# Amanda-Zheng/MR-GNAS

Measured on AMD Instinct MI355X. Metric: million edges/sec per supernet fwd+bwd step (FB15k-237, dim=200), higher is better.
Workload: dtype f32

## Files before the change

### include/mrgnas.h

```cpp
#ifndef MRGNAS_H
#define MRGNAS_H

#include <stdint.h>

#ifdef __cplusplus
extern "C" {
#endif

#define MRG_ABI_VERSION 23

#define MRG_OK            0
#define MRG_E_NULLPTR    -1
#define MRG_E_SHAPE      -2
#define MRG_E_ENUM       -3
#define MRG_E_WORKSPACE  -4

#define MRG_COMPOSE_MULT 0
#define MRG_COMPOSE_SUB  1
#define MRG_COMPOSE_ADD  2
#define MRG_REDUCE_SUM   0
#define MRG_REDUCE_MEAN  1
#define MRG_REDUCE_MAX   2
#define MRG_GCS_SUB      0
#define MRG_GCS_MUL      1
// ... 31 lines not shown
int mrg_gate_fwd(const float *s, const float *s_in, const float *norm, const float *uvc,
                 float *out, int64_t b0, int64_t b1, int64_t M, int D, float scale, void *stream);
int64_t mrg_gate_bwd_workspace_bytes(int64_t M, int D);
int mrg_gate_bwd(const float *gout, const float *s, const float *s_in, const float *norm,
                 const float *uvc, float *gs, float *gs_in, float *d_uvc, void *ws,
                 int64_t b0, int64_t b1, int64_t M, int D, float scale, void *stream);
int mrg_gate_row_fwd(const float *s, const float *s_in, const float *norm, const float *uvc, float *fvec, float *hvec,
                     int64_t b0, int64_t b1, int64_t M, int D, float scale, void *stream);
int64_t mrg_gate_row_colsum_blocks(int64_t b0, int64_t b1, int64_t M, int D, int vec4);
int mrg_gate_row_fwd_colsum(const float *s, const float *s_in, const float *norm, const float *uvc, float *fvec, float *hvec,
                            int64_t b0, int64_t b1, int64_t M, int D, float scale, void *stream, double *colsum, int64_t colsum_blocks);
int mrg_gate_row_bwd(const float *q, const float *hvec, const float *s, const float *s_in, const float *uvc, float *gs_in, float *d_uvc,
                     void *ws, int64_t b0, int64_t b1, int64_t M, int D, void *stream);
int mrg_gate_row_bwd_acc(const float *q, const float *hvec, const float *s, const float *s_in, const float *uvc, float *gs_in, float *d_uvc,
                         void *ws, int64_t b0, int64_t b1, int64_t M, int D, void *stream, const float *total);

int64_t mrg_seg_reduce_workspace_bytes(int64_t n_slots, int D);
int mrg_seg_reduce_fwd(int mode, const float *msg, const float *self_rows,
                       const int32_t *eid,
                       const int32_t *chunk_node, const int32_t *chunk_start, const int32_t *chunk_end,
                       const int32_t *chunk_slot, int64_t n_chunks,
                       const int32_t *hub_node, const int32_t *hub_first, const int32_t *hub_count, int64_t n_hubs,
                       int64_t n_slots, const int32_t *in_degree,
                       float *out, int32_t *arg, void *ws,
                       int64_t N, int D, void *stream);
int mrg_seg_reduce_bwd(int mode, const float *gout, const int32_t *dst, const int32_t *in_degree,
                       const int32_t *arg, float *gmsg, float *gself, const float *relu_src,
                       int64_t E, int64_t N, int D, void *stream);
int mrg_seg_reduce_bwd_ordered(int mode, const float *gout, const int32_t *dst, const int32_t *in_degree, const int32_t *arg,
                               float *gmsg, float *gself, const float *relu_src, const unsigned *relu_bits, const int32_t *order,
// ... 144 lines not shown
                                 int64_t b0, int64_t b1, int64_t M, int D, void *stream, double *colsum, int64_t colsum_blocks);
int mrg_dense_filter_dz3(int kind, const float *g, const float *s, const float *gate, const float *norm, float scale_edge,
                         float scale_self, float *dz, float *gs, int64_t b1, int64_t M, int D, void *stream);
int64_t mrg_linear_bwd_input3_workspace_bytes(int K, int Nout);
int mrg_linear_bwd_input3(const float *gY, const float *const *W, float *gX, void *ws, int64_t b0, int64_t b1, int64_t M,
                          int K, int Nout, int ldw, int accumulate, void *stream);
int64_t mrg_linear_bwd_input3_pair_workspace_bytes(int K, int Nout);
int mrg_linear_bwd_input3_pair(const float *gY1, const float *gY2, const float *const *W1, const float *const *W2, float *gX,
                               void *ws, int64_t b0, int64_t b1, int64_t M, int K, int Nout, int ldw, int accumulate,
                               void *stream);
int mrg_linear_bwd_input3_acc2(const float *gY, const float *const *W, float *gX, void *ws, int64_t b0, int64_t b1, int64_t M,
                               int K, int Nout, int ldw, int accumulate, void *stream, const float *total);
int mrg_linear_bwd_input3_pair_acc2(const float *gY1, const float *gY2, const float *const *W1, const float *const *W2, float *gX,
                                    void *ws, int64_t b0, int64_t b1, int64_t M, int K, int Nout, int ldw, int accumulate,
                                    void *stream, const float *total);
int64_t mrg_linear_bwd_weight3_workspace_bytes(int64_t b0, int64_t b1, int64_t M, int K1, int K2, int Nout);
int mrg_linear_bwd_weight3(const float *gY, const float *X1, const float *X2, float *const *gW, float *const *gbias, void *ws,
                           int64_t b0, int64_t b1, int64_t M, int K1, int K2, int Nout, void *stream);
int mrg_dense_filter_dz(int kind, const float *g, const float *s, const float *gate, const float *rowscale,
                        float scale, float *dz, float *gs, int64_t rows, int D, void *stream);

int64_t mrg_build_graph_workspace_bytes(int64_t T);
int mrg_build_graph(const int64_t *triples, int64_t T, int64_t N, int R, int sorted,
                    const float *deg_norm_table, int64_t table_len,
                    int64_t *src, int64_t *dst, int64_t *etype, float *norm, int32_t *in_degree,
                    int32_t *src32, int32_t *dst32, int32_t *etype32, int32_t *max_degree,
                    void *ws, int64_t ws_bytes, void *stream);

int64_t mrg_plan_workspace_bytes(int64_t E, int64_t nseg, int span);
int mrg_span_plan_build(const int32_t *seg, int64_t E, int64_t nseg, int span, int snap,
// ... 176 lines not shown
```

### mr-gnas_amd/_lib.py

```python
import ctypes
import os
import re

import torch

_HERE = os.path.dirname(os.path.abspath(__file__))
LIB_PATH = os.environ.get("MRG_LIB_PATH") or os.path.join(_HERE, "lib", "libmrgnas_hip.so")
HEADER_PATH = os.path.join(os.path.dirname(_HERE), "include", "mrgnas.h")

ABI_VERSION = 23


class MrgnasLibraryError(RuntimeError):
    pass


class MrgnasError(RuntimeError):
    """A C-ABI call returned a non-zero code."""


_P, _I, _L, _F = ctypes.c_void_p, ctypes.c_int, ctypes.c_int64, ctypes.c_float

SIGNATURES = {
    "mrg_abi_version": (_I, []),
# ... 10 lines not shown
    "mrg_gate_bwd_workspace_bytes": (_L, [_L, _I]),
    "mrg_gate_bwd": (_I, [_P, _P, _P, _P, _P, _P, _P, _P, _P, _L, _L, _L, _I, _F, _P]),
    "mrg_seg_reduce_workspace_bytes": (_L, [_L, _I]),
    "mrg_seg_reduce_fwd": (_I, [_I, _P, _P, _P, _P, _P, _P, _P, _L, _P, _P, _P, _L, _L, _P, _P, _P, _P, _L, _I, _P]),
    "mrg_seg_reduce_bwd": (_I, [_I, _P, _P, _P, _P, _P, _P, _P, _L, _L, _I, _P]),
    "mrg_fused_gcs": (_I, [_I, _P, _P, _P, _P, _P, _P, _P, _P, _P, _P, _L, _P, _P, _P, _L, _L, _P, _P, _P, _L, _I, _P]),
    "mrg_span_gcs": (_I, [_I, _P, _P, _P, _P, _L, _I, _P, _P, _L, _P, _P, _P, _L, _L, _P, _P, _P, _L, _I, _P]),
    "mrg_sum_buffers": (_I, [_P, _I, _P, _L, _I, _P]),
    "mrg_sum_rows_gather": (_I, [_P, _I, _P, _P, _P, _L, _L, _I, _P, _P]),
    "mrg_distmult_score": (_I, [_P, _P, _P, _P, _P, _P, _L, _I, _P]),
    "mrg_gate_row_fwd": (_I, [_P, _P, _P, _P, _P, _P, _L, _L, _L, _I, _F, _P]),
    "mrg_gate_row_colsum_blocks": (_L, [_L, _L, _L, _I, _I]),
    "mrg_gate_row_fwd_colsum": (_I, [_P, _P, _P, _P, _P, _P, _L, _L, _L, _I, _F, _P, _P, _L]),
    "mrg_gate_row_bwd": (_I, [_P, _P, _P, _P, _P, _P, _P, _P, _L, _L, _L, _I, _P]),
    "mrg_gate_row_bwd_acc": (_I, [_P, _P, _P, _P, _P, _P, _P, _P, _L, _L, _L, _I, _P, _P]),
    "mrg_mix_workspace_bytes": (_L, [_I, _I]),
    "mrg_mix_colstats": (_I, [_P, _I, _L, _I, _P, _P, _P, _P]),
    "mrg_mix_finalize_fwd": (_I, [_P, _P, _P, _P, _P, _I, ctypes.c_double, _I, _F, _F, _P, _P]),
    "mrg_mix_stats_coef": (_I, [_P, _P, _P, _P, _P, _I, _L, ctypes.c_double, _I, _F, _F, _P, _P, _P, _P]),
    "mrg_zero_workspace_bytes": (_L, [_I]),
    "mrg_zero_colstats": (_I, [_P, _P, _P, _P, _P, _I, _L, _I, _P, _P, _P]),
    "mrg_zero_stats_coef": (_I, [_P, _P, _P, _P, _P, _I, _P, _P, _P, _P, _L, ctypes.c_double, _I, _F, _F, _P, _P, _P, _P]),
    "mrg_zero_fwd": (_I, [_P, _P, _P, _P, _P, _I, _P, _P, _P, _L, _I, _P, _P]),
    "mrg_zero_bwd_reduce": (_I, [_P, _P, _P, _P, _P, _P, _I, _P, _P, _P, _P, _L, _I, _P, _P]),
    "mrg_zero_bwd_apply": (_I, [_P, _P, _P, _P, _P, _P, _I, _P, _P, _P, _P, _P, _L, _I, _P, _P]),
    "mrg_mix_fwd": (_I, [_P, _I, _P, _P, _P, _P, _L, _I, _P, _P]),
    "mrg_mix_bwd_reduce": (_I, [_P, _P, _I, _P, _P, _P, _P, _L, _I, _P, _P]),
    "mrg_mix_finalize_bwd": (_I, [_P, _I, ctypes.c_double, _I, _P, _P, _P, _P, _P, _P]),
    "mrg_mix_bwd_apply": (_I, [_P, _P, _P, _I, _P, _P, _P, _P, _P, _P, _P, _P, _P, _P, _P, _P, _P, _L, _I, _P, _P]),
    "mrg_dense_filter_fwd": (_I, [_I, _P, _P, _P, _P, _P, _F, _P, _P, _P, _L, _I, _P]),
# ... 14 lines not shown
    "mrg_adam_step": (_I, [_P, _P, _P, _P, _L, _P, _P, _P, _L, _P, _P, _P, ctypes.c_double, ctypes.c_double, _F, _F, _P]),
    "mrg_act_grad_transpose": (_I, [_P, _P, _P, _L, _L, _I, _P]),
    "mrg_wgrad_set_variant": (_I, [_I]),
    "mrg_linear_fwd": (_I, [_P, _P, _P, _P, _P, _L, _I, _I, _I, _P]),
    "mrg_dense_filter3_workspace_bytes": (_L, [_I, _I]),
    "mrg_dense_filter_fwd3": (_I, [_I, _P, _P, _P, _P, _P, _F, _F, _P, _P, _P, _L, _L, _L, _I, _P]),
    "mrg_dense_filter3_colsum_blocks": (_L, [_I, _L, _L, _L, _I, _I]),
    "mrg_dense_filter_fwd3_colsum": (_I, [_I, _P, _P, _P, _P, _P, _F, _F, _P, _P, _P, _L, _L, _L, _I, _P, _P, _L]),
    "mrg_dense_filter_dz3": (_I, [_I, _P, _P, _P, _P, _F, _F, _P, _P, _L, _L, _I, _P]),
    "mrg_linear_bwd_input3_workspace_bytes": (_L, [_I, _I]),
    "mrg_linear_bwd_input3": (_I, [_P, _P, _P, _P, _L, _L, _L, _I, _I, _I, _I, _P]),
    "mrg_linear_bwd_input3_acc2": (_I, [_P, _P, _P, _P, _L, _L, _L, _I, _I, _I, _I, _P, _P]),
    "mrg_linear_bwd_input3_pair_workspace_bytes": (_L, [_I, _I]),
    "mrg_linear_bwd_input3_pair": (_I, [_P, _P, _P, _P, _P, _P, _L, _L, _L, _I, _I, _I, _I, _P]),
    "mrg_linear_bwd_input3_pair_acc2": (_I, [_P, _P, _P, _P, _P, _P, _L, _L, _L, _I, _I, _I, _I, _P, _P]),
    "mrg_linear_bwd_weight3_workspace_bytes": (_L, [_L, _L, _L, _I, _I, _I]),
    "mrg_linear_bwd_weight3": (_I, [_P, _P, _P, _P, _P, _P, _L, _L, _L, _I, _I, _I, _P]),
    "mrg_linear_relu_segsum_fwd": (_I, [_P, _P, _P, _P, _P, _P, _P, _P, _L, _I, _I, _P]),
    "mrg_seg_reduce_heads_fwd": (_I, [_I, _P, _P, _P, _P, _P, _P, _P, _L, _P, _P, _P, _L, _L, _P, _P, _P, _L, _I, _P]),
    "mrg_seg_reduce_bwd_bits": (_I, [_I, _P, _P, _P, _P, _P, _P, _L, _L, _I, _P]),
    "mrg_seg_reduce_bwd_ordered": (_I, [_I, _P, _P, _P, _P, _P, _P, _P, _P, _P, _L, _L, _I, _P]),
    "mrg_linear_relu_segmax_workspace_bytes": (_L, [_L, _I, _I]),
    "mrg_linear_relu_segmax_fwd": (_I, [_P, _P, _P, _P, _P, _P, _P, _P, _P, _P, _L, _L, _I, _I, _P]),
    "mrg_linear_bwd_input_workspace_bytes": (_L, [_I, _I]),
    "mrg_linear_bwd_input": (_I, [_P, _P, _P, _P, _L, _I, _I, _I, _I, _P]),
    "mrg_linear_bwd_input_acc2": (_I, [_P, _P, _P, _P, _L, _I, _I, _I, _I, _P, _P]),
    "mrg_linear_bwd_weight_workspace_bytes": (_L, [_L, _I, _I]),
    "mrg_linear_bwd_weight": (_I, [_P, _P, _P, _P, _P, _P, _L, _I, _I, _I, _P]),
    "mrg_linear_bwd_weight_share": (_I, [_P, _P, _P, _P, _P, _P, _L, _I, _I, _I, _I, _P]),
    "mrg_build_graph_workspace_bytes": (_L, [_L]),
# ... 255 lines not shown
```

### mr-gnas_amd/csrc/gate.hip

```cpp
#include "common.hpp"

namespace mrg {

struct SegPlan {
  int64_t lo[3], hi[3];
  int blk[4];
};

static SegPlan make_plan(int64_t b0, int64_t b1, int64_t M, int grid) {
  SegPlan p;
  p.lo[0] = 0;  p.hi[0] = b0;
  p.lo[1] = b0; p.hi[1] = b1;
  p.lo[2] = b1; p.hi[2] = M;
  int nseg = 0;
  for (int s = 0; s < 3; ++s) nseg += (p.hi[s] > p.lo[s]);
  int spare = grid - nseg;
  p.blk[0] = 0;
  for (int s = 0; s < 3; ++s) {
    int64_t rows = p.hi[s] - p.lo[s];
    int nb = rows > 0 ? 1 + (int)((double)spare * (double)rows / (double)M) : 0;
    p.blk[s + 1] = p.blk[s] + nb;
  }
  return p;
}
// ... 362 lines not shown
  float* mine = red + rw * (2 * WIDTH + 1);
#pragma unroll
  for (int k = 0; k < KMAX; ++k) {
    int c = sl + k * LPR;
#pragma unroll
    for (int j = 0; j < VEC; ++j) {
      mine[c * VEC + j] = du[k][j];
      mine[WIDTH + c * VEC + j] = dvv[k][j];
    }
  }
  if (sl == 0) mine[2 * WIDTH] = (float)dc;
  __syncthreads();
  float* dst = ws + (int64_t)b * ld;
  for (int t = threadIdx.x; t < ld; t += MRG_BLOCK) {
    int srcidx = t < D ? t : ((HAS_IN && t < 2 * D) ? WIDTH + (t - D) : (t == cidx ? 2 * WIDTH : -1));
    double acc = 0.0;
    if (srcidx >= 0) {
#pragma unroll
      for (int q = 0; q < RPB; ++q) acc += (double)red[q * (2 * WIDTH + 1) + srcidx];
    }
    dst[t] = (float)acc;
  }
}

__global__ void gate_reduce_k(const float* __restrict__ ws, float* __restrict__ d_uvc, SegPlan p, int ld) {
  int seg = blockIdx.y;
  int t = blockIdx.x * blockDim.x + threadIdx.x;
  if (t >= ld) return;
  double acc = 0.0;
  for (int b = p.blk[seg]; b < p.blk[seg + 1]; ++b) acc += (double)ws[(int64_t)b * ld + t];
// ... 230 lines not shown
extern "C" int64_t mrg_gate_row_colsum_blocks(int64_t b0, int64_t b1, int64_t M, int D, int vec4) {
  if (D <= 0 || M <= 0 || b0 < 0 || b1 < b0 || M < b1) return 0;
  RowGeom g = row_geom(D, vec4 != 0);
  if (!g.ok || g.kmax != 1 || (vec4 && g.vec != 4)) return 0;
  SegPlan p;
  return gate_row_plan(b0, b1, M, g.lpr, &p);
}

extern "C" int mrg_gate_row_fwd_colsum(const float* s, const float* s_in, const float* norm, const float* uvc, float* fvec, float* hvec,
                                       int64_t b0, int64_t b1, int64_t M, int D, float scale, void* stream, double* colsum, int64_t colsum_blocks) {
  if (!colsum) return MRG_E_NULLPTR;
  return gate_row_fwd(s, s_in, norm, uvc, fvec, hvec, b0, b1, M, D, scale, stream, colsum, colsum_blocks);
}

static int gate_row_bwd(const float* q, const float* hvec, const float* s, const float* s_in, const float* uvc, float* gs_in, float* d_uvc,
                        void* ws, int64_t b0, int64_t b1, int64_t M, int D, void* stream, const float* total) {
  if (D <= 0 || M < 0 || b0 < 0 || b1 < b0 || M < b1) return MRG_E_SHAPE;
  if (!uvc || !d_uvc) return MRG_E_NULLPTR;
  if (M > 0 && (!q || !hvec || !s)) return MRG_E_NULLPTR;
  if (s_in && !gs_in) return MRG_E_NULLPTR;
  if (total && !s_in) return MRG_E_NULLPTR;
  if (!ws) return MRG_E_WORKSPACE;
  hipStream_t st = (hipStream_t)stream;
  const int ld = MRG_GATE_LD(D);
  RowGeom g = row_geom(D, aligned16(s) && aligned16(s_in) && aligned16(gs_in) && aligned16(uvc) && aligned16(total));
  if (!g.ok) return MRG_E_SHAPE;
  SegPlan p{};
#define CALL(V, L, K)                                                                                                   \
  do {                                                                                                                  \
    int grid = grid_for(M, (MRG_BLOCK / L) * 4);                                                                        \
    if (grid < 3) grid = 3;                                                                                             \
    p = make_plan(b0, b1, M, grid);                                                                                     \
    if (M > 0) {                                                                                                        \
      if (total) hipLaunchKernelGGL((gate_row_bwd_k<V, L, K, true, true>), dim3(p.blk[3]), dim3(MRG_BLOCK), 0, st, q, hvec, s, s_in, uvc, gs_in, (float*)ws, p, D, total); \
      else if (s_in) hipLaunchKernelGGL((gate_row_bwd_k<V, L, K, true>), dim3(p.blk[3]), dim3(MRG_BLOCK), 0, st, q, hvec, s, s_in, uvc, gs_in, (float*)ws, p, D, nullptr); \
      else hipLaunchKernelGGL((gate_row_bwd_k<V, L, K, false>), dim3(p.blk[3]), dim3(MRG_BLOCK), 0, st, q, hvec, s, s_in, uvc, gs_in, (float*)ws, p, D, nullptr); \
    }                                                                                                                   \
  } while (0)
  MRG_DISPATCH_GEOM(g, CALL);
#undef CALL
  MRG_LAUNCH_CHECK();
  launch_ordered_reduce_ranges<float>((const float*)ws, d_uvc, p.blk, 3, ld, ld, ld, st);
  MRG_LAUNCH_CHECK();
  return MRG_OK;
}

extern "C" int mrg_gate_row_bwd(const float* q, const float* hvec, const float* s, const float* s_in, const float* uvc, float* gs_in, float* d_uvc,
                                void* ws, int64_t b0, int64_t b1, int64_t M, int D, void* stream) {
  return gate_row_bwd(q, hvec, s, s_in, uvc, gs_in, d_uvc, ws, b0, b1, M, D, stream, nullptr);
}

extern "C" int mrg_gate_row_bwd_acc(const float* q, const float* hvec, const float* s, const float* s_in, const float* uvc, float* gs_in, float* d_uvc,
                                    void* ws, int64_t b0, int64_t b1, int64_t M, int D, void* stream, const float* total) {
  if (!total) return MRG_E_NULLPTR;
  return gate_row_bwd(q, hvec, s, s_in, uvc, gs_in, d_uvc, ws, b0, b1, M, D, stream, total);
}
```

### mr-gnas_amd/csrc/gemm.hpp

```cpp
#pragma once
#include "common.hpp"

namespace mrg {

typedef float f32x16 __attribute__((ext_vector_type(16)));
typedef float v4f __attribute__((ext_vector_type(4)));
typedef __attribute__((address_space(3))) void* lds_ptr_t;
typedef const __attribute__((address_space(1))) void* gbl_ptr_t;

constexpr int GBM_MAX = 256;

enum { EPI_BIAS_ACT = 0, EPI_GATE = 1, EPI_SCALE = 2, EPI_ACCUM = 3, EPI_SEGMAX = 4, EPI_SEGSUM = 5 };
enum { EPI_GATE_SUMS = 6, EPI_SCALE_SUMS = 7 };
constexpr bool epi_sums(int epi) { return epi == EPI_GATE_SUMS || epi == EPI_SCALE_SUMS; }
constexpr int epi_base(int epi) { return epi == EPI_GATE_SUMS ? EPI_GATE : (epi == EPI_SCALE_SUMS ? EPI_SCALE : epi); }
enum { EPI_RANK = 8, EPI_RANK_DIAG = 9 };
constexpr bool epi_diag(int epi) { return epi == EPI_RANK_DIAG; }
enum { EPI_BCE = 10, EPI_BCE_GRAD = 11 };
enum { EPI_ACCUM2 = 12 };
constexpr bool epi_accum(int epi) { return epi == EPI_ACCUM || epi == EPI_ACCUM2; }
enum { EPI_TOPK = 13 };
enum { EPI_BCE_BIAS = 14, EPI_BCE_GRAD_BIAS = 15, EPI_RANK_BIAS = 16, EPI_TOPK_BIAS = 17 };
constexpr bool epi_col_bias(int epi) { return epi >= EPI_BCE_BIAS && epi <= EPI_TOPK_BIAS; }
constexpr int epi_unbiased(int epi) {
  return epi == EPI_BCE_BIAS ? EPI_BCE : (epi == EPI_BCE_GRAD_BIAS ? EPI_BCE_GRAD : (epi == EPI_RANK_BIAS ? EPI_RANK : (epi == EPI_TOPK_BIAS ? EPI_TOPK : epi)));
}
struct GemmArgs;
template <int NT>
__device__ __forceinline__ void gemm_epilogue_topk(const GemmArgs& a, f32x16 (&acc)[NT], int64_t rowbase, int col0, int li, int lh);

struct GemmGroups {
  int n;
  int tile0[4];
  int64_t lo[3], hi[3];
  int64_t bp_stride;
  const float* bias[3];
  float scale[3];
  int use_rowscale[3];
};
inline int gemm_group_tiles(GemmGroups& g, int gbm) {
// ... 829 lines not shown
```

### mr-gnas_amd/csrc/gemm_x3q.hpp

```cpp
#pragma once
#include "gemm_x3.hpp"

namespace mrg {

constexpr int X3Q_CHUNK = X3Q_HT * 3 * 1024;
constexpr int X3Q_ROWS = 64;

inline size_t x3q_bsplit_bytes(int K) { return (size_t)x3q_slabs(K) * 2 * X3Q_CHUNK; }

template <int EPI, bool SUMS = false>
__device__ __forceinline__ void gemm_epilogue_q(const GemmArgs& a, f32x4v (&acc)[X3Q_NT], int64_t rowbase, int li, int lh, bool full,
                                                double* __restrict__ sums = nullptr) {
  static_assert(!SUMS || EPI == EPI_GATE || EPI == EPI_SCALE, "column sums: gate and scale epilogues only");
  constexpr int W = X3Q_HT * 32;
  if (rowbase >= a.rows) {
    if constexpr (SUMS) {
#pragma unroll
      for (int j = 0; j < X3Q_HT; ++j) { sums[(lh * 2 + 0) * W + j * 32 + li] = 0.0; sums[(lh * 2 + 1) * W + j * 32 + li] = 0.0; }
    }
    return;
  }
  const int last = (int)((a.rows - 1 - rowbase) < 15 ? (a.rows - 1 - rowbase) : 15);
  const int colw = li < a.N ? li : a.N - 1;
  float* crow[8];
// ... 3 lines not shown
  float cs[8];
  bool rok[8];
  const bool cstore = EPI != EPI_GATE || a.C != nullptr;
#pragma unroll
  for (int i = 0; i < 8; ++i) {
    const int row = i + 8 * lh;
    const int rc = row < last ? row : last;
    rok[i] = row <= last;
    crow[i] = a.C + (rowbase + rc) * a.ldc + colw;
    if (EPI == EPI_GATE) srow[i] = a.S + (rowbase + rc) * a.ld_s + colw;
    if (epi_accum(EPI)) srow[i] = a.Cin + (rowbase + rc) * a.ld_cin + colw;
    if (EPI == EPI_ACCUM2) trow[i] = a.S + (rowbase + rc) * a.ld_s + colw;
    if (EPI == EPI_GATE) xrow[i] = a.aux ? a.aux + (rowbase + rc) * a.N + colw : nullptr;
    cs[i] = 1.0f;
    if (EPI == EPI_GATE || EPI == EPI_SCALE) cs[i] = a.scale * (a.rowscale ? a.rowscale[rowbase + rc] : 1.0f);
  }
  const int lc = li & 15;
#pragma unroll
  for (int j = 0; j < X3Q_HT; ++j) {
    const int ca = (2 * j) * 16 + lc, cb = (2 * j + 1) * 16 + lc;
    const float bva = a.bias ? a.bias[ca < a.N ? ca : a.N - 1] : 0.f;
    const float bvb = a.bias ? a.bias[cb < a.N ? cb : a.N - 1] : 0.f;
    float acc8[8];
#pragma unroll
    for (int r = 0; r < 4; ++r) {
      float xa = acc[2 * j][r] + bva, xb = acc[2 * j + 1][r] + bvb;
      asm volatile("s_nop 1\n\tv_permlane16_swap_b32 %0, %1" : "+v"(xa), "+v"(xb));
      acc8[r] = xa;
      acc8[4 + r] = xb;
    }
    const int col = j * 32 + li;
    const bool cok = col < a.N;
    const int off = cok ? j * 32 : 0;
    float in[8], in2[8], v[8], g[8];
#pragma unroll
    for (int i = 0; i < 8; ++i) in[i] = 0.f;
    if ((EPI == EPI_GATE && (cstore || SUMS)) || epi_accum(EPI)) {
#pragma unroll
      for (int i = 0; i < 8; ++i) in[i] = srow[i][off];
    }
    if (EPI == EPI_ACCUM2) {
#pragma unroll
      for (int i = 0; i < 8; ++i) in2[i] = trow[i][off];
    }
#pragma unroll
    for (int i = 0; i < 8; ++i) {
      const float x = acc8[i];
      if (EPI == EPI_BIAS_ACT) {
        v[i] = (a.act == MRG_ACT_RELU) ? (x > 0.f ? x : 0.f) : (a.act == MRG_ACT_SIGMOID ? sigmoidf_fast(x) : x);
      } else if (EPI == EPI_GATE) {
        g[i] = sigmoidf_fast(x);
        v[i] = g[i] * in[i] * cs[i];
      } else if (EPI == EPI_ACCUM2) {
        v[i] = (x + in[i]) + in2[i];
      } else if (EPI == EPI_SCALE) {
        v[i] = x * cs[i];
      } else {
        v[i] = x + in[i];
      }
    }
    if constexpr (SUMS) {
      double s1 = 0.0, s2 = 0.0;
#pragma unroll
      for (int i = 0; i < 8; ++i) {
        const double d = (full || rok[i]) ? (double)v[i] : 0.0;
        s1 += d; s2 += d * d;
      }
      sums[(lh * 2 + 0) * W + j * 32 + li] = cok ? s1 : 0.0;
      sums[(lh * 2 + 1) * W + j * 32 + li] = cok ? s2 : 0.0;
    }
    if (full) {
// ... 146 lines not shown
```

### mr-gnas_amd/csrc/linear.hip

```cpp
#include "gemm_dispatch.hpp"

namespace mrg {

__global__ void segmax_finalize_k(const unsigned long long* __restrict__ keys, const float* __restrict__ self_rows,
                                  const int32_t* __restrict__ eid, float* __restrict__ out, int32_t* __restrict__ arg,
                                  float* __restrict__ mx, int64_t total) {
  for (int64_t i = (int64_t)blockIdx.x * blockDim.x + threadIdx.x; i < total; i += (int64_t)gridDim.x * blockDim.x) {
    const unsigned long long k = keys[i];
    const unsigned lo = (unsigned)k;
    const float v = __uint_as_float((unsigned)(k >> 32));
    out[i] = self_rows ? v + self_rows[i] : v;
    if (arg) arg[i] = lo == 0u ? -1 : eid[0xFFFFFFFFu - lo];
    if (mx) mx[i] = v;
  }
}

}

using namespace mrg;

static bool segmax_shape_ok(int K, int Nout) { return K > 48 && K % 4 == 0 && Nout > 0; }

extern "C" int64_t mrg_linear_relu_segmax_workspace_bytes(int64_t N, int K, int Nout) {
  if (N < 0 || !segmax_shape_ok(K, Nout) || gemm_mode() == 1) return 0;
// ... 117 lines not shown
  if (!ws) return MRG_E_WORKSPACE;
  hipStream_t st = (hipStream_t)stream;
  GemmArgs a{};
  a.A1 = gY; a.K1 = Nout; a.B = W; a.C = gX; a.ldc = K; a.N = K; a.rows = rows; a.act = MRG_ACT_NONE;
  if (accumulate) {
    a.Cin = gX; a.ld_cin = K;
    gemm_set_cin2(a, total, K);
    return launch_gemm<EPI_ACCUM2>(a, 1, ldw, ws, st);
  }
  a.Cin = total; a.ld_cin = K;
  return launch_gemm<EPI_ACCUM>(a, 1, ldw, ws, st);
}

static size_t bwd_input3_each(int K, int Nred) { return (size_t)(((int64_t)bsplit_bytes_any(K, Nred) + 255) / 256 * 256); }

static int bwd_input3(const float* gY1, const float* gY2, const float* const* W1_host, const float* const* W2_host, float* gX, void* ws,
                      int64_t b0, int64_t b1, int64_t M, int K, int Nout, int ldw, int accumulate, hipStream_t st,
                      const float* total = nullptr) {
  const bool pair = gY2 != nullptr;
  const int Nred = pair ? 2 * Nout : Nout;
  GemmArgs a{};
  a.A1 = gY1; a.K1 = Nout; a.C = gX; a.ldc = K; a.N = K; a.rows = M; a.act = MRG_ACT_NONE;
  if (pair) { a.A2 = gY2; a.K2 = Nout; }
  if (accumulate) { a.Cin = gX; a.ld_cin = K; }
  if (total && accumulate) {
    if (total == gX) return MRG_E_SHAPE;
    gemm_set_cin2(a, total, K);
  } else if (total) {
    a.Cin = total; a.ld_cin = K;
  }
  const int epi = total && accumulate ? EPI_ACCUM2 : (total || accumulate ? EPI_ACCUM : EPI_BIAS_ACT);
  if (!x3_eligible(a)) return MRG_E_SHAPE;
  const int64_t lo[3] = {0, b0, b1}, hi[3] = {b0, b1, M};
  const size_t each = bwd_input3_each(K, Nred);
// ... 52 lines not shown
  if (M == 0) return MRG_OK;
  if (!gY1 || !gY2 || !W1_host || !W2_host || !gX) return MRG_E_NULLPTR;
  if (!ws) return MRG_E_WORKSPACE;
  return bwd_input3(gY1, gY2, W1_host, W2_host, gX, ws, b0, b1, M, K, Nout, ldw, accumulate, (hipStream_t)stream);
}

extern "C" int mrg_linear_bwd_input3_pair_acc2(const float* gY1, const float* gY2, const float* const* W1_host, const float* const* W2_host, float* gX,
                                               void* ws, int64_t b0, int64_t b1, int64_t M, int K, int Nout, int ldw, int accumulate, void* stream,
                                               const float* total) {
  if (K <= 0 || Nout <= 24 || Nout % 4 != 0 || ldw < K || M < 0 || b0 < 0 || b1 < b0 || M < b1) return MRG_E_SHAPE;
  if (M == 0) return MRG_OK;
  if (!gY1 || !gY2 || !W1_host || !W2_host || !gX || !total) return MRG_E_NULLPTR;
  if (!ws) return MRG_E_WORKSPACE;
  return bwd_input3(gY1, gY2, W1_host, W2_host, gX, ws, b0, b1, M, K, Nout, ldw, accumulate, (hipStream_t)stream, total);
}
```

### mr-gnas_amd/functional/dense.py

```python
import weakref

import torch

from .. import _lib
from .._lib import ptr_array, call, f32c, ptr, require_hip, stream_of
from . import switches as SW
from ._base import Fork, _ws, _ws_bytes, same_rows
from .candidates import Candidate, Link, RowScale, wants_stats
from .fanin import Fan, join


def _bwd_input3(name, head, tail, gX, accumulate, jn, **work):
    st = stream_of(gX if gX is not None else jn.total)
    if jn is None or jn.total is None:
        call(name, (*head, ptr(gX), *tail, accumulate, st), **work)
        if jn is None:
            return gX
        jn.deposit(gX)
        return None
    tot = jn.total
    out = gX if accumulate else tot
    work["nbytes"] = work.get("nbytes", 0) + 4 * tot.numel()
    call(name, (*head, ptr(out), *tail, accumulate, st, ptr(tot)), **work)
    jn.deposit(out)
# ... 225 lines not shown
            dz_d, gs = torch.empty_like(s), torch.empty_like(s)
            call("mrg_dense_filter_dz3", (0, ptr(g_d), ptr(s), ptr(gate), ptr(norm), 1.0 / 3.0, 1.0 / 3.0, ptr(dz_d), ptr(gs), b1, M, D, st),
                 nbytes=4 * M * D * 5)
        if pres[1]:
            dz_c = g_c
        else:
            dz_c = torch.empty_like(s)
            call("mrg_dense_filter_dz3", (1, ptr(g_c), ptr(s), None, ptr(norm), 1.0 / 3.0, 1.0, ptr(dz_c), None, b1, M, D, st), nbytes=4 * M * D * 2)
        lib = _lib.load()
        wsp = int(lib.mrg_linear_bwd_input3_pair_workspace_bytes(D, D))
        gwork = dict(nbytes=4 * M * 3 * D + 24 * D * D, flops=4 * M * D * D)
        gs = _bwd_input3("mrg_linear_bwd_input3_pair", (ptr(dz_d), ptr(dz_c), ptr_array(dW), ptr_array(cW)), (ptr(_ws(wsp, s)), b0, b1, M, D, D, K_),
                         gs, 1, join(ctx.fan[0], s), nbytes=4 * M * 4 * D + 24 * D * D, flops=4 * M * D * D)
        gs_in = None
        if s_in is not None:
            jn = join(ctx.fan[1], s)
            gs_in = torch.empty_like(s) if (jn is None or jn.total is None) else None
            gs_in = _bwd_input3("mrg_linear_bwd_input3_pair", (ptr(dz_d), ptr(dz_c), ptr_array([W[:, D:] for W in dW]), ptr_array([W[:, D:] for W in cW])),
                                (ptr(_ws(wsp, s)), b0, b1, M, D, D, K_), gs_in, 0, jn, **gwork)
        wsw = int(lib.mrg_linear_bwd_weight3_workspace_bytes(b0, b1, M, D, K_ - D, D))
        g_dW = [torch.empty_like(W) for W in dW]
        g_dB = [torch.empty_like(params[2 * i + 1]) for i in range(3)]
        g_cW = [torch.empty_like(W) for W in cW]
        wwork = dict(nbytes=4 * M * (D + K_), flops=2 * M * K_ * D)
        call("mrg_linear_bwd_weight3", (ptr(dz_d), ptr(s), ptr(s_in), ptr_array(g_dW), ptr_array(g_dB), ptr(_ws(wsw, s)), b0, b1, M, D, K_ - D, D, st), **wwork)
        call("mrg_linear_bwd_weight3", (ptr(dz_c), ptr(s), ptr(s_in), ptr_array(g_cW), ptr_array([None, None, None]), ptr(_ws(wsw, s)), b0, b1, M, D, K_ - D, D, st),
             **wwork)
        grads_d = [t for pair in zip(g_dW, g_dB) for t in pair]
        return (None, None, gs, gs_in, None, None, None, None, *grads_d, *g_cW)


def dense_pair_available(D, tied):
    if not (SW.DENSE_PAIR and SW.GROUPED_SEGMENTS):
        return False
# ... 62 lines not shown
```

### mr-gnas_amd/functional/fanin.py

```python
import weakref

import torch

from .._lib import ptr_array, call, f32c, ptr, require_hip, stream_of
from . import switches as SW
from .reducers import _seg_bwd


def sum_buffers(xs):
    xs = [f32c(x) for x in xs]
    require_hip(*xs)
    out = torch.empty_like(xs[0])
    n = out.numel()
    for i in range(0, len(xs), 8):
        part = xs[i:i + 8]
        call("mrg_sum_buffers", (ptr_array(part), len(part), ptr(out), n, int(i > 0), stream_of(out)),
             nbytes=4 * n * (len(part) + 1 + int(i > 0)))
    return out


class _Fanout(torch.autograd.Function):

    @staticmethod
    def forward(ctx, x, k, box):
# ... 43 lines not shown
        if not gs[0].is_cuda or any(g.shape != gs[0].shape for g in gs):
            out = gs[0]
            for g in gs[1:]:
                out = out + g
            return out
        return sum_buffers(gs)


_RAW_STREAM = torch._C._cuda_getCurrentRawStream


def _graph_task():
    return torch._C._current_graph_task_id()


class _FanBox:
    __slots__ = ("gathered", "total", "spent")

    def __init__(self):
        self.gathered = None
        self.total = None
        self.spent = False

    def take_total(self, like):
        if self.total is None:
            return None
        buf, stream, task = self.total
        if task != _graph_task():
            self.total = None
            return None
        if like is not None and (buf.shape != like.shape or buf.device != like.device or buf.dtype != like.dtype):
            return None
        self.total = None
        if stream is not None and _RAW_STREAM(buf.get_device()) != stream:
            cur = torch.cuda.current_stream(buf.device)
            ev = torch.cuda.Event()
            ev.record(torch.cuda.ExternalStream(stream, device=buf.device))
            cur.wait_event(ev)
            buf.record_stream(cur)
        return buf

    def deposit(self, buf):
        self.total = (buf, _RAW_STREAM(buf.get_device()) if buf.is_cuda else None, _graph_task())


class _Join:
    __slots__ = ("box", "total")

    def __init__(self, box, total):
        self.box, self.total = box, total

    def deposit(self, buf):
        self.box.deposit(buf)


def join(box, like, absorbs_gather=False):
    if box is None or not SW.FANIN_CHAIN or box.spent or not like.is_cuda or torch.is_grad_enabled() or _graph_task() < 0:
        return None
    if box.gathered is not None and not absorbs_gather:
        return None
    tot = box.take_total(like)
    if tot is None and box.total is not None:
        return None
    return _Join(box, tot)


class Fan:

    BATCH = 12

    def __init__(self, x, cap):
        self.x = x
        self.left = cap
        self._live = torch.is_grad_enabled() and x.requires_grad and cap > 1
        self._views = []
        self._root = x
# ... 28 lines not shown
```

### mr-gnas_amd/functional/gates.py

```python
import torch

from .. import _lib
from .._lib import ptr_array, call, f32c, ptr, require_hip, stream_of
from ._base import _ws, _ws_bytes, gate_ld, same_rows
from .candidates import Candidate, Link, wants_stats
from .fanin import Fan, join


class _Gate(torch.autograd.Function):

    @staticmethod
    def forward(ctx, s, s_in, norm, b0, b1, scale, *params):
        tied = s_in is not None and same_rows(s, s_in)
        s, s_in, norm = f32c(s), (None if tied else f32c(s_in)), f32c(norm)
        params = tuple(f32c(p) for p in params)
        require_hip(s, s_in, norm, *params)
        M, D = s.shape
        st = stream_of(s)
        in_dim = 2 * D if (s_in is not None or tied) else D
        Ws, bs, as_ = params[0::3], params[1::3], params[2::3]
        uvc = torch.empty(3, gate_ld(D), dtype=torch.float32, device=s.device)
        call("mrg_gate_collapse3", (ptr_array(Ws), ptr_array(bs), ptr_array(as_), ptr(uvc), D, in_dim, int(tied), st),
             nbytes=4 * D * in_dim * sum(W is not None for W in Ws))
        out = torch.empty_like(s)
# ... 69 lines not shown
        ctx.cfg = (b0, b1, scale, in_dim, tied)
        ctx.link = link
        if link is not None:
            link.row_h, link.row_uvc = hvec, uvc
        return fvec

    @staticmethod
    def backward(ctx, gq):
        s, s_in, norm, uvc, hvec, *params = ctx.saved_tensors
        b0, b1, scale, in_dim, tied = ctx.cfg
        gq = f32c(gq)
        M, D = s.shape
        st = stream_of(s)
        jn = join(ctx.fan_in, s) if s_in is not None else None
        tot = jn.total if jn is not None else None
        gs_in = tot if tot is not None else (torch.empty_like(s) if s_in is not None else None)
        d_uvc = torch.empty(3, gate_ld(D), dtype=torch.float32, device=s.device)
        ws = _ws(_ws_bytes("mrg_gate_bwd_workspace_bytes", M, D), s)
        nb = 4 * D * M * (3 if s_in is not None else 1) + 8 * M
        args = (ptr(gq), ptr(hvec), ptr(s), ptr(s_in), ptr(uvc), ptr(gs_in), ptr(d_uvc), ptr(ws), b0, b1, M, D, st)
        if tot is not None:
            call("mrg_gate_row_bwd", args + (ptr(tot),), nbytes=nb + 4 * D * M)
        else:
            call("mrg_gate_row_bwd", args, nbytes=nb)
        if jn is not None:
            jn.deposit(gs_in)
            gs_in = None
        Ws, bs, as_ = params[0::3], params[1::3], params[2::3]
        gWs = [None if W is None else torch.empty_like(W) for W in Ws]
        gbs = [None if b is None else torch.empty_like(b) for b in bs]
        gas = [None if a is None else torch.empty_like(a) for a in as_]
        call("mrg_gate_param_grad3", (ptr_array(Ws), ptr_array(bs), ptr_array(as_), ptr(d_uvc), ptr_array(gWs), ptr_array(gbs), ptr_array(gas),
                                      D, in_dim, int(tied), st), nbytes=8 * D * in_dim * sum(W is not None for W in Ws))
        gparams = []
        for gW, gb, ga in zip(gWs, gbs, gas):
            gparams += [gW, gb, ga]
# ... 24 lines not shown
```

### mr-gnas_amd/functional/switches.py

```python
import os

ROW_FACTOR = os.environ.get("MRG_ROW_FACTOR", "1") == "1"
LAZY_ASUM = os.environ.get("MRG_LAZY_ASUM", "1") == "1"
FANIN_CHAIN = os.environ.get("MRG_FANIN_CHAIN", "1") == "1"
FUSED_AMAX = os.environ.get("MRG_FUSED_AMAX", "1") == "1"
FUSED_AMAX_MIN_ROWS = int(os.environ.get("MRG_FUSED_AMAX_MIN_ROWS", "100000"))
FUSED_AMEAN = os.environ.get("MRG_FUSED_AMEAN", "1") == "1"
WIDE_BWD_INPUT = os.environ.get("MRG_WIDE_BWD_INPUT", "1") == "1"
NODE_LINEAR = os.environ.get("MRG_NODE_LINEAR", "1") == "1"
MASK_TAP = None
FOLD_IDENTITY = os.environ.get("MRG_FOLD_IDENTITY", "1") == "1"
CELL_ZERO_FUSED = os.environ.get("MRG_CELL_ZERO_FUSED", "1") == "1"
FORK_MIN_ROWS = int(os.environ.get("MRG_FORK_MIN_ROWS", str(1 << 17)))
SEGMENT_STREAMS = int(os.environ.get("MRG_SEGMENT_STREAMS", "3"))
FOLD_ROW_SCALE = os.environ.get("MRG_FOLD_ROW_SCALE", "1") == "1"
GROUPED_SEGMENTS = os.environ.get("MRG_GROUPED_SEGMENTS", "1") == "1"
DENSE_PAIR = os.environ.get("MRG_DENSE_PAIR", "1") == "1"
GATED_RECOMPUTE = os.environ.get("MRG_GATED_RECOMPUTE", "1") == "1"
PRODUCER_STATS = os.environ.get("MRG_PRODUCER_STATS", "1") == "1"
COMPGCN_TAIL = os.environ.get("MRG_COMPGCN_TAIL", "1") == "1"
SPARSE_AMAX_BWD = os.environ.get("MRG_SPARSE_AMAX_BWD", "1") == "1"
CAND_LINEAR_GROUP = os.environ.get("MRG_CAND_LINEAR_GROUP", "1") == "1"
CCORR_PATH = None
```

Measured before the change: 11.93.

## Defer row-gate input gradient as rank-1 factor folded into dense bwd GEMM epilogue

The row-factor gate backward now writes only the per-row dz vector and a lazy Rank1 handle instead of materialising the full M×D gradient for s_in. When the downstream dense filter's pair input-gradient GEMM is the consumer and the plan matches, the GEMM epilogue adds dz[r]*uvc[col] directly, avoiding one full-size write and a later read of the gradient. If the consumer cannot absorb the rank-1 form, the fill closure recomputes the full gradient with an extra kernel. This adds complexity in the fan-in chain, stream bookkeeping and a new epilogue mode.

After: 11.92. Within noise of the previous version (-0.1%).

```diff
diff --git a/include/mrgnas.h b/include/mrgnas.h
--- a/include/mrgnas.h
+++ b/include/mrgnas.h
@@ -69,6 +69,8 @@
                      void *ws, int64_t b0, int64_t b1, int64_t M, int D, void *stream);
 int mrg_gate_row_bwd_acc(const float *q, const float *hvec, const float *s, const float *s_in, const float *uvc, float *gs_in, float *d_uvc,
                          void *ws, int64_t b0, int64_t b1, int64_t M, int D, void *stream, const float *total);
+int mrg_gate_row_bwd_dz(const float *q, const float *hvec, const float *s, const float *s_in, const float *uvc, float *dz, float *d_uvc,
+                        void *ws, int64_t b0, int64_t b1, int64_t M, int D, void *stream);
 
 int64_t mrg_seg_reduce_workspace_bytes(int64_t n_slots, int D);
 int mrg_seg_reduce_fwd(int mode, const float *msg, const float *self_rows,
@@ -243,6 +245,10 @@
 int mrg_linear_bwd_input3_pair_acc2(const float *gY1, const float *gY2, const float *const *W1, const float *const *W2, float *gX,
                                     void *ws, int64_t b0, int64_t b1, int64_t M, int K, int Nout, int ldw, int accumulate,
                                     void *stream, const float *total);
+int mrg_linear_bwd_input3_rank1_ok(int64_t M, int K, int Nred);
+int mrg_linear_bwd_input3_pair_rank1(const float *gY1, const float *gY2, const float *const *W1, const float *const *W2, float *gX,
+                                     void *ws, int64_t b0, int64_t b1, int64_t M, int K, int Nout, int ldw, void *stream,
+                                     const float *dz, const float *uvc);
 int64_t mrg_linear_bwd_weight3_workspace_bytes(int64_t b0, int64_t b1, int64_t M, int K1, int K2, int Nout);
 int mrg_linear_bwd_weight3(const float *gY, const float *X1, const float *X2, float *const *gW, float *const *gbias, void *ws,
                            int64_t b0, int64_t b1, int64_t M, int K1, int K2, int Nout, void *stream);
diff --git a/mr-gnas_amd/_lib.py b/mr-gnas_amd/_lib.py
--- a/mr-gnas_amd/_lib.py
+++ b/mr-gnas_amd/_lib.py
@@ -48,6 +48,7 @@
     "mrg_gate_row_fwd_colsum": (_I, [_P, _P, _P, _P, _P, _P, _L, _L, _L, _I, _F, _P, _P, _L]),
     "mrg_gate_row_bwd": (_I, [_P, _P, _P, _P, _P, _P, _P, _P, _L, _L, _L, _I, _P]),
     "mrg_gate_row_bwd_acc": (_I, [_P, _P, _P, _P, _P, _P, _P, _P, _L, _L, _L, _I, _P, _P]),
+    "mrg_gate_row_bwd_dz": (_I, [_P, _P, _P, _P, _P, _P, _P, _P, _L, _L, _L, _I, _P]),
     "mrg_mix_workspace_bytes": (_L, [_I, _I]),
     "mrg_mix_colstats": (_I, [_P, _I, _L, _I, _P, _P, _P, _P]),
     "mrg_mix_finalize_fwd": (_I, [_P, _P, _P, _P, _P, _I, ctypes.c_double, _I, _F, _F, _P, _P]),
@@ -92,6 +93,8 @@
     "mrg_linear_bwd_input3_pair_workspace_bytes": (_L, [_I, _I]),
     "mrg_linear_bwd_input3_pair": (_I, [_P, _P, _P, _P, _P, _P, _L, _L, _L, _I, _I, _I, _I, _P]),
     "mrg_linear_bwd_input3_pair_acc2": (_I, [_P, _P, _P, _P, _P, _P, _L, _L, _L, _I, _I, _I, _I, _P, _P]),
+    "mrg_linear_bwd_input3_rank1_ok": (_I, [_L, _I, _I]),
+    "mrg_linear_bwd_input3_pair_rank1": (_I, [_P, _P, _P, _P, _P, _P, _L, _L, _L, _I, _I, _I, _P, _P, _P]),
     "mrg_linear_bwd_weight3_workspace_bytes": (_L, [_L, _L, _L, _I, _I, _I]),
     "mrg_linear_bwd_weight3": (_I, [_P, _P, _P, _P, _P, _P, _L, _L, _L, _I, _I, _I, _P]),
     "mrg_linear_relu_segsum_fwd": (_I, [_P, _P, _P, _P, _P, _P, _P, _P, _L, _I, _I, _P]),
diff --git a/mr-gnas_amd/csrc/gate.hip b/mr-gnas_amd/csrc/gate.hip
--- a/mr-gnas_amd/csrc/gate.hip
+++ b/mr-gnas_amd/csrc/gate.hip
@@ -400,6 +400,69 @@
   float* dst = ws + (int64_t)b * ld;
   for (int t = threadIdx.x; t < ld; t += MRG_BLOCK) {
     int srcidx = t < D ? t : ((HAS_IN && t < 2 * D) ? WIDTH + (t - D) : (t == cidx ? 2 * WIDTH : -1));
+    double acc = 0.0;
+    if (srcidx >= 0) {
+#pragma unroll
+      for (int q = 0; q < RPB; ++q) acc += (double)red[q * (2 * WIDTH + 1) + srcidx];
+    }
+    dst[t] = (float)acc;
+  }
+}
+
+template <int VEC, int LPR, int KMAX>
+__global__ __launch_bounds__(MRG_BLOCK) void gate_row_bwd_dz_k(const float* __restrict__ qv, const float* __restrict__ hv, const float* __restrict__ s,
+                                                               const float* __restrict__ sin_, float* __restrict__ dzout,
+                                                               float* __restrict__ ws, SegPlan p, int D) {
+  constexpr int RPB = MRG_BLOCK / LPR;
+  constexpr int WIDTH = LPR * KMAX * VEC;
+  __shared__ float red[RPB * (2 * WIDTH + 1)];
+  const int b = blockIdx.x;
+  if (b >= p.blk[3]) return;
+  const int seg = (b >= p.blk[1]) + (b >= p.blk[2]);
+  const int jb = b - p.blk[seg], nb = p.blk[seg + 1] - p.blk[seg];
+  const int sl = threadIdx.x % LPR, rw = row_group_of_thread<LPR>();
+  const int dv = D / VEC;
+  const int ld = MRG_GATE_LD(D);
+  const int cidx = 2 * D;
+  Vec<VEC> du[KMAX], dvv[KMAX];
+  double dc = 0.0;
+#pragma unroll
+  for (int k = 0; k < KMAX; ++k) {
+    du[k] = Vec<VEC>::fill(0.f);
+    dvv[k] = Vec<VEC>::fill(0.f);
+  }
+  for (int64_t r = p.lo[seg] + (int64_t)jb * RPB + rw; r < p.hi[seg]; r += (int64_t)nb * RPB) {
+    const float dz = qv[r] * hv[r];
+    dc += (double)dz;
+    if (sl == 0) dzout[r] = dz;
+#pragma unroll
+    for (int k = 0; k < KMAX; ++k) {
+      int c = sl + k * LPR;
+      if (c < dv) {
+        const Vec<VEC> sk = Vec<VEC>::load(s + r * D + c * VEC);
+#pragma unroll
+        for (int j = 0; j < VEC; ++j) du[k][j] += dz * sk[j];
+        const Vec<VEC> xk = Vec<VEC>::load(sin_ + r * D + c * VEC);
+#pragma unroll
+        for (int j = 0; j < VEC; ++j) dvv[k][j] += dz * xk[j];
+      }
+    }
+  }
+  float* mine = red + rw * (2 * WIDTH + 1);
+#pragma unroll
+  for (int k = 0; k < KMAX; ++k) {
+    int c = sl + k * LPR;
+#pragma unroll
+    for (int j = 0; j < VEC; ++j) {
+      mine[c * VEC + j] = du[k][j];
+      mine[WIDTH + c * VEC + j] = dvv[k][j];
+    }
+  }
+  if (sl == 0) mine[2 * WIDTH] = (float)dc;
+  __syncthreads();
+  float* dst = ws + (int64_t)b * ld;
+  for (int t = threadIdx.x; t < ld; t += MRG_BLOCK) {
+    int srcidx = t < D ? t : (t < 2 * D ? WIDTH + (t - D) : (t == cidx ? 2 * WIDTH : -1));
     double acc = 0.0;
     if (srcidx >= 0) {
 #pragma unroll
@@ -660,12 +723,13 @@
 }
 
 static int gate_row_bwd(const float* q, const float* hvec, const float* s, const float* s_in, const float* uvc, float* gs_in, float* d_uvc,
-                        void* ws, int64_t b0, int64_t b1, int64_t M, int D, void* stream, const float* total) {
+                        void* ws, int64_t b0, int64_t b1, int64_t M, int D, void* stream, const float* total, float* dz_out = nullptr) {
   if (D <= 0 || M < 0 || b0 < 0 || b1 < b0 || M < b1) return MRG_E_SHAPE;
   if (!uvc || !d_uvc) return MRG_E_NULLPTR;
   if (M > 0 && (!q || !hvec || !s)) return MRG_E_NULLPTR;
-  if (s_in && !gs_in) return MRG_E_NULLPTR;
+  if (s_in && !gs_in && !dz_out) return MRG_E_NULLPTR;
   if (total && !s_in) return MRG_E_NULLPTR;
+  if (dz_out && (!s_in || total || gs_in)) return MRG_E_NULLPTR;
   if (!ws) return MRG_E_WORKSPACE;
   hipStream_t st = (hipStream_t)stream;
   const int ld = MRG_GATE_LD(D);
@@ -678,7 +742,8 @@
     if (grid < 3) grid = 3;                                                                                             \
     p = make_plan(b0, b1, M, grid);                                                                                     \
     if (M > 0) {                                                                                                        \
-      if (total) hipLaunchKernelGGL((gate_row_bwd_k<V, L, K, true, true>), dim3(p.blk[3]), dim3(MRG_BLOCK), 0, st, q, hvec, s, s_in, uvc, gs_in, (float*)ws, p, D, total); \
+      if (dz_out) hipLaunchKernelGGL((gate_row_bwd_dz_k<V, L, K>), dim3(p.blk[3]), dim3(MRG_BLOCK), 0, st, q, hvec, s, s_in, dz_out, (float*)ws, p, D); \
+      else if (total) hipLaunchKernelGGL((gate_row_bwd_k<V, L, K, true, true>), dim3(p.blk[3]), dim3(MRG_BLOCK), 0, st, q, hvec, s, s_in, uvc, gs_in, (float*)ws, p, D, total); \
       else if (s_in) hipLaunchKernelGGL((gate_row_bwd_k<V, L, K, true>), dim3(p.blk[3]), dim3(MRG_BLOCK), 0, st, q, hvec, s, s_in, uvc, gs_in, (float*)ws, p, D, nullptr); \
       else hipLaunchKernelGGL((gate_row_bwd_k<V, L, K, false>), dim3(p.blk[3]), dim3(MRG_BLOCK), 0, st, q, hvec, s, s_in, uvc, gs_in, (float*)ws, p, D, nullptr); \
     }                                                                                                                   \
@@ -701,3 +766,9 @@
   if (!total) return MRG_E_NULLPTR;
   return gate_row_bwd(q, hvec, s, s_in, uvc, gs_in, d_uvc, ws, b0, b1, M, D, stream, total);
 }
+
+extern "C" int mrg_gate_row_bwd_dz(const float* q, const float* hvec, const float* s, const float* s_in, const float* uvc, float* dz, float* d_uvc,
+                                   void* ws, int64_t b0, int64_t b1, int64_t M, int D, void* stream) {
+  if (!dz || !s_in) return MRG_E_NULLPTR;
+  return gate_row_bwd(q, hvec, s, s_in, uvc, nullptr, d_uvc, ws, b0, b1, M, D, stream, nullptr, dz);
+}
diff --git a/mr-gnas_amd/csrc/gemm.hpp b/mr-gnas_amd/csrc/gemm.hpp
--- a/mr-gnas_amd/csrc/gemm.hpp
+++ b/mr-gnas_amd/csrc/gemm.hpp
@@ -24,6 +24,12 @@
 constexpr bool epi_col_bias(int epi) { return epi >= EPI_BCE_BIAS && epi <= EPI_TOPK_BIAS; }
 constexpr int epi_unbiased(int epi) {
   return epi == EPI_BCE_BIAS ? EPI_BCE : (epi == EPI_BCE_GRAD_BIAS ? EPI_BCE_GRAD : (epi == EPI_RANK_BIAS ? EPI_RANK : (epi == EPI_TOPK_BIAS ? EPI_TOPK : epi)));
+}
+enum { EPI_RANK1 = 18 };
+__device__ __forceinline__ float gemm_rank1_add(float x, float r, float v) {
+#pragma clang fp contract(off)
+  const float p = r * v;
+  return x + p;
 }
 struct GemmArgs;
 template <int NT>
diff --git a/mr-gnas_amd/csrc/gemm_x3q.hpp b/mr-gnas_amd/csrc/gemm_x3q.hpp
--- a/mr-gnas_amd/csrc/gemm_x3q.hpp
+++ b/mr-gnas_amd/csrc/gemm_x3q.hpp
@@ -41,13 +41,14 @@
     if (EPI == EPI_GATE) xrow[i] = a.aux ? a.aux + (rowbase + rc) * a.N + colw : nullptr;
     cs[i] = 1.0f;
     if (EPI == EPI_GATE || EPI == EPI_SCALE) cs[i] = a.scale * (a.rowscale ? a.rowscale[rowbase + rc] : 1.0f);
+    if (EPI == EPI_RANK1) cs[i] = a.rowscale[rowbase + rc];
   }
   const int lc = li & 15;
 #pragma unroll
   for (int j = 0; j < X3Q_HT; ++j) {
     const int ca = (2 * j) * 16 + lc, cb = (2 * j + 1) * 16 + lc;
-    const float bva = a.bias ? a.bias[ca < a.N ? ca : a.N - 1] : 0.f;
-    const float bvb = a.bias ? a.bias[cb < a.N ? cb : a.N - 1] : 0.f;
+    const float bva = (EPI != EPI_RANK1 && a.bias) ? a.bias[ca < a.N ? ca : a.N - 1] : 0.f;
+    const float bvb = (EPI != EPI_RANK1 && a.bias) ? a.bias[cb < a.N ? cb : a.N - 1] : 0.f;
     float acc8[8];
 #pragma unroll
     for (int r = 0; r < 4; ++r) {
@@ -70,6 +71,8 @@
 #pragma unroll
       for (int i = 0; i < 8; ++i) in2[i] = trow[i][off];
     }
+    float vcol = 0.f;
+    if (EPI == EPI_RANK1) vcol = a.bias[cok ? col : colw];
 #pragma unroll
     for (int i = 0; i < 8; ++i) {
       const float x = acc8[i];
@@ -82,6 +85,8 @@
         v[i] = (x + in[i]) + in2[i];
       } else if (EPI == EPI_SCALE) {
         v[i] = x * cs[i];
+      } else if (EPI == EPI_RANK1) {
+        v[i] = gemm_rank1_add(x, cs[i], vcol);
       } else {
         v[i] = x + in[i];
       }
diff --git a/mr-gnas_amd/csrc/linear.hip b/mr-gnas_amd/csrc/linear.hip
--- a/mr-gnas_amd/csrc/linear.hip
+++ b/mr-gnas_amd/csrc/linear.hip
@@ -155,10 +155,42 @@
 
 static size_t bwd_input3_each(int K, int Nred) { return (size_t)(((int64_t)bsplit_bytes_any(K, Nred) + 255) / 256 * 256); }
 
+extern "C" int mrg_linear_bwd_input3_rank1_ok(int64_t M, int K, int Nred) {
+  if (M <= X3N_MAX_ROWS || K <= 0 || Nred <= 48 || Nred % 8 != 0) return 0;
+  return x3q_shape(EPI_RANK1, K, Nred) ? 1 : 0;
+}
+
 static int bwd_input3(const float* gY1, const float* gY2, const float* const* W1_host, const float* const* W2_host, float* gX, void* ws,
                       int64_t b0, int64_t b1, int64_t M, int K, int Nout, int ldw, int accumulate, hipStream_t st,
-                      const float* total = nullptr) {
+                      const float* total = nullptr, const float* r1_dz = nullptr, const float* r1_uvc = nullptr) {
   const bool pair = gY2 != nullptr;
+  if (r1_dz) {
+    if (!pair || accumulate || total || !r1_uvc) return MRG_E_SHAPE;
+    if (!mrg_linear_bwd_input3_rank1_ok(M, K, 2 * Nout)) return MRG_E_SHAPE;
+    GemmArgs a{};
+    a.A1 = gY1; a.K1 = Nout; a.A2 = gY2; a.K2 = Nout; a.C = gX; a.ldc = K; a.N = K; a.rows = M; a.act = MRG_ACT_NONE;
+    a.rowscale = r1_dz;
+    if (!x3q_eligible(a)) return MRG_E_SHAPE;
+    const int64_t lo[3] = {0, b0, b1}, hi[3] = {b0, b1, M};
+    const size_t each = bwd_input3_each(K, 2 * Nout);
+    const float* Bs[3]; const float* Bs2[3]; void* outs[3];
+    a.grp.n = 3;
+    a.grp.bp_stride = (int64_t)each;
+    for (int i = 0; i < 3; ++i) {
+      const bool live = hi[i] > lo[i];
+      if (live && (!W1_host[i] || !W2_host[i])) return MRG_E_NULLPTR;
+      Bs[i] = live ? W1_host[i] : nullptr;
+      Bs2[i] = live ? W2_host[i] : nullptr;
+      outs[i] = (char*)ws + i * each;
+      a.grp.lo[i] = lo[i]; a.grp.hi[i] = live ? hi[i] : lo[i];
+      a.grp.scale[i] = 1.0f;
+      a.grp.use_rowscale[i] = 1;
+      a.grp.bias[i] = r1_uvc + (int64_t)i * MRG_GATE_LD(K) + K;
+    }
+    launch_bsplit3_any(EPI_RANK1, M, Bs, 1, ldw, K, 2 * Nout, outs, st, Bs2, Nout);
+    MRG_LAUNCH_CHECK();
+    return launch_rowgemm_x3q<EPI_RANK1>(a, outs[0], st);
+  }
   const int Nred = pair ? 2 * Nout : Nout;
   GemmArgs a{};
   a.A1 = gY1; a.K1 = Nout; a.C = gX; a.ldc = K; a.N = K; a.rows = M; a.act = MRG_ACT_NONE;
@@ -241,3 +273,13 @@
   if (!ws) return MRG_E_WORKSPACE;
   return bwd_input3(gY1, gY2, W1_host, W2_host, gX, ws, b0, b1, M, K, Nout, ldw, accumulate, (hipStream_t)stream, total);
 }
+
+extern "C" int mrg_linear_bwd_input3_pair_rank1(const float* gY1, const float* gY2, const float* const* W1_host, const float* const* W2_host, float* gX,
+                                                void* ws, int64_t b0, int64_t b1, int64_t M, int K, int Nout, int ldw, void* stream,
+                                                const float* dz, const float* uvc) {
+  if (K <= 0 || Nout <= 24 || Nout % 4 != 0 || ldw < K || M < 0 || b0 < 0 || b1 < b0 || M < b1) return MRG_E_SHAPE;
+  if (M == 0) return MRG_OK;
+  if (!gY1 || !gY2 || !W1_host || !W2_host || !gX || !dz || !uvc) return MRG_E_NULLPTR;
+  if (!ws) return MRG_E_WORKSPACE;
+  return bwd_input3(gY1, gY2, W1_host, W2_host, gX, ws, b0, b1, M, K, Nout, ldw, 0, (hipStream_t)stream, nullptr, dz, uvc);
+}
diff --git a/mr-gnas_amd/functional/dense.py b/mr-gnas_amd/functional/dense.py
--- a/mr-gnas_amd/functional/dense.py
+++ b/mr-gnas_amd/functional/dense.py
@@ -7,7 +7,7 @@
 from . import switches as SW
 from ._base import Fork, _ws, _ws_bytes, same_rows
 from .candidates import Candidate, Link, RowScale, wants_stats
-from .fanin import Fan, join
+from .fanin import Fan, Rank1, join
 
 
 def _bwd_input3(name, head, tail, gX, accumulate, jn, **work):
@@ -263,10 +263,20 @@
                          gs, 1, join(ctx.fan[0], s), nbytes=4 * M * 4 * D + 24 * D * D, flops=4 * M * D * D)
         gs_in = None
         if s_in is not None:
-            jn = join(ctx.fan[1], s)
-            gs_in = torch.empty_like(s) if (jn is None or jn.total is None) else None
-            gs_in = _bwd_input3("mrg_linear_bwd_input3_pair", (ptr(dz_d), ptr(dz_c), ptr_array([W[:, D:] for W in dW]), ptr_array([W[:, D:] for W in cW])),
-                                (ptr(_ws(wsp, s)), b0, b1, M, D, D, K_), gs_in, 0, jn, **gwork)
+            jn = join(ctx.fan[1], s, rank1=True)
+            tot = jn.total if jn is not None else None
+            head = (ptr(dz_d), ptr(dz_c), ptr_array([W[:, D:] for W in dW]), ptr_array([W[:, D:] for W in cW]))
+            if isinstance(tot, Rank1) and tot.plan == (b0, b1) and bool(lib.mrg_linear_bwd_input3_rank1_ok(M, D, 2 * D)):
+                gs_in = torch.empty_like(s)
+                call("mrg_linear_bwd_input3_pair", (*head, ptr(gs_in), ptr(_ws(wsp, s)), b0, b1, M, D, D, K_, st, ptr(tot.dz), ptr(tot.uvc)),
+                     symbol="mrg_linear_bwd_input3_pair_rank1", nbytes=gwork["nbytes"] + 4 * M, flops=gwork["flops"])
+                jn.deposit(gs_in)
+                gs_in = None
+            else:
+                if isinstance(tot, Rank1):
+                    jn.total = tot.materialise()
+                gs_in = torch.empty_like(s) if (jn is None or jn.total is None) else None
+                gs_in = _bwd_input3("mrg_linear_bwd_input3_pair", head, (ptr(_ws(wsp, s)), b0, b1, M, D, D, K_), gs_in, 0, jn, **gwork)
         wsw = int(lib.mrg_linear_bwd_weight3_workspace_bytes(b0, b1, M, D, K_ - D, D))
         g_dW = [torch.empty_like(W) for W in dW]
         g_dB = [torch.empty_like(params[2 * i + 1]) for i in range(3)]
diff --git a/mr-gnas_amd/functional/fanin.py b/mr-gnas_amd/functional/fanin.py
--- a/mr-gnas_amd/functional/fanin.py
+++ b/mr-gnas_amd/functional/fanin.py
@@ -81,6 +81,24 @@
     return torch._C._current_graph_task_id()
 
 
+class Rank1:
+    __slots__ = ("dz", "uvc", "plan", "shape", "device", "dtype", "fill")
+
+    def __init__(self, dz, uvc, plan, shape, fill):
+        self.dz, self.uvc, self.plan, self.shape, self.fill = dz, uvc, plan, torch.Size(shape), fill
+        self.device, self.dtype = dz.device, dz.dtype
+
+    @property
+    def is_cuda(self):
+        return self.dz.is_cuda
+
+    def get_device(self):
+        return self.dz.get_device()
+
+    def materialise(self):
+        return self.fill()
+
+
 class _FanBox:
     __slots__ = ("gathered", "total", "spent")
 
@@ -89,7 +107,7 @@
         self.total = None
         self.spent = False
 
-    def take_total(self, like):
+    def take_total(self, like, rank1=False):
         if self.total is None:
             return None
         buf, stream, task = self.total
@@ -99,12 +117,17 @@
         if like is not None and (buf.shape != like.shape or buf.device != like.device or buf.dtype != like.dtype):
             return None
         self.total = None
-        if stream is not None and _RAW_STREAM(buf.get_device()) != stream:
+        is_r1 = isinstance(buf, Rank1)
+        other = stream is not None and _RAW_STREAM(buf.get_device()) != stream
+        if other:
             cur = torch.cuda.current_stream(buf.device)
             ev = torch.cuda.Event()
             ev.record(torch.cuda.ExternalStream(stream, device=buf.device))
             cur.wait_event(ev)
-            buf.record_stream(cur)
+            for t in ((buf.dz, buf.uvc) if is_r1 else (buf,)):
+                t.record_stream(cur)
+        if is_r1 and (other or not rank1):
+            buf = buf.materialise()
         return buf
 
     def deposit(self, buf):
@@ -121,12 +144,12 @@
         self.box.deposit(buf)
 
 
-def join(box, like, absorbs_gather=False):
+def join(box, like, absorbs_gather=False, rank1=False):
     if box is None or not SW.FANIN_CHAIN or box.spent or not like.is_cuda or torch.is_grad_enabled() or _graph_task() < 0:
         return None
     if box.gathered is not None and not absorbs_gather:
         return None
-    tot = box.take_total(like)
+    tot = box.take_total(like, rank1)
     if tot is None and box.total is not None:
         return None
     return _Join(box, tot)
diff --git a/mr-gnas_amd/functional/gates.py b/mr-gnas_amd/functional/gates.py
--- a/mr-gnas_amd/functional/gates.py
+++ b/mr-gnas_amd/functional/gates.py
@@ -4,7 +4,8 @@
 from .._lib import ptr_array, call, f32c, ptr, require_hip, stream_of
 from ._base import _ws, _ws_bytes, gate_ld, same_rows
 from .candidates import Candidate, Link, wants_stats
-from .fanin import Fan, join
+from . import switches as SW
+from .fanin import Fan, Rank1, join
 
 
 class _Gate(torch.autograd.Function):
@@ -107,12 +108,24 @@
         st = stream_of(s)
         jn = join(ctx.fan_in, s) if s_in is not None else None
         tot = jn.total if jn is not None else None
-        gs_in = tot if tot is not None else (torch.empty_like(s) if s_in is not None else None)
+        rank1 = (jn is not None and tot is None and SW.FANIN_RANK1 and bool(_lib.load().mrg_linear_bwd_input3_rank1_ok(M, D, 2 * D)))
+        gs_in = tot if tot is not None else (torch.empty_like(s) if (s_in is not None and not rank1) else None)
         d_uvc = torch.empty(3, gate_ld(D), dtype=torch.float32, device=s.device)
         ws = _ws(_ws_bytes("mrg_gate_bwd_workspace_bytes", M, D), s)
         nb = 4 * D * M * (3 if s_in is not None else 1) + 8 * M
         args = (ptr(gq), ptr(hvec), ptr(s), ptr(s_in), ptr(uvc), ptr(gs_in), ptr(d_uvc), ptr(ws), b0, b1, M, D, st)
-        if tot is not None:
+        if rank1:
+            dz = torch.empty(M, dtype=torch.float32, device=s.device)
+            call("mrg_gate_row_bwd", args[:5] + (ptr(dz),) + args[6:], nbytes=nb - 4 * D * M + 4 * M, symbol="mrg_gate_row_bwd_dz")
+
+            def fill():
+                out, scratch = torch.empty_like(s), torch.empty_like(d_uvc)
+                ws2 = _ws(_ws_bytes("mrg_gate_bwd_workspace_bytes", M, D), s)
+                call("mrg_gate_row_bwd", (ptr(gq), ptr(hvec), ptr(s), ptr(s_in), ptr(uvc), ptr(out), ptr(scratch), ptr(ws2), b0, b1, M, D,
+                                          stream_of(s)), nbytes=nb)
+                return out
+            gs_in = Rank1(dz, uvc, (b0, b1), s.shape, fill)
+        elif tot is not None:
             call("mrg_gate_row_bwd", args + (ptr(tot),), nbytes=nb + 4 * D * M)
         else:
             call("mrg_gate_row_bwd", args, nbytes=nb)
diff --git a/mr-gnas_amd/functional/switches.py b/mr-gnas_amd/functional/switches.py
--- a/mr-gnas_amd/functional/switches.py
+++ b/mr-gnas_amd/functional/switches.py
@@ -3,6 +3,7 @@
 ROW_FACTOR = os.environ.get("MRG_ROW_FACTOR", "1") == "1"
 LAZY_ASUM = os.environ.get("MRG_LAZY_ASUM", "1") == "1"
 FANIN_CHAIN = os.environ.get("MRG_FANIN_CHAIN", "1") == "1"
+FANIN_RANK1 = os.environ.get("MRG_FANIN_RANK1", "1") == "1"
 FUSED_AMAX = os.environ.get("MRG_FUSED_AMAX", "1") == "1"
 FUSED_AMAX_MIN_ROWS = int(os.environ.get("MRG_FUSED_AMAX_MIN_ROWS", "100000"))
 FUSED_AMEAN = os.environ.get("MRG_FUSED_AMEAN", "1") == "1"
```
